# b41sh/pa

Measured on AMD Instinct MI355X. Metric: decoded GB/s (uncompressed) per node at 1/2/4/8 GPUs; bit-exact vs CPU, higher is better.
Workload: dtype int32

## Files before the change

include/strawboat_gpu.h:

```cpp
#ifndef STRAWBOAT_GPU_H
#define STRAWBOAT_GPU_H

#include <stddef.h>
#include <stdint.h>

#ifdef __cplusplus
extern "C" {
#endif

typedef enum {
  SB_OK = 0,
  SB_E_OUT_OF_SPEC = 1,
  SB_E_NYI = 2,
  SB_E_IO = 3,
  SB_E_CODEC = 4,
  SB_E_DEVICE = 5,
  SB_E_ARG = 6,
} sb_status;

typedef enum {
  SB_CODEC_NONE = 0,
  SB_CODEC_LZ4 = 1,
  SB_CODEC_ZSTD = 2,
  SB_CODEC_SNAPPY = 3,
// ... 222 lines not shown
                                       const sb_write_options* opts, uint64_t max_page_rows, uint8_t* d_out,
                                       uint64_t out_capacity, uint64_t* out_len, sb_page_meta* h_metas,
                                       uint64_t metas_cap, uint64_t* n_pages);
typedef struct {
  const int64_t* d_offsets;
  const uint8_t* d_validity;
} sb_nest_dev;
uint64_t sb_encode_nested_device_bound(const sb_nested_desc* desc, uint64_t n_rows, uint64_t n_level_bound,
                                       uint64_t n_leaf, uint64_t values_len, uint64_t max_page_rows);
sb_status sb_encode_nested_column_device(sb_ctx* ctx, const sb_nested_desc* desc, const sb_nest_dev* d_nests,
                                         const void* d_values, const int64_t* d_leaf_offsets, uint64_t values_len,
                                         const uint8_t* d_leaf_validity, uint64_t n_rows,
                                         const sb_write_options* opts, uint64_t max_page_rows, uint8_t* d_out,
                                         uint64_t out_capacity, uint64_t* out_len, sb_page_meta* h_metas,
                                         uint64_t metas_cap, uint64_t* n_pages);
sb_status sb_write_footer(const uint8_t* h_schema, uint64_t schema_len, const uint64_t* h_col_offsets,
                          const uint64_t* h_col_npages, uint64_t n_cols, const sb_page_meta* h_pages,
                          uint8_t** h_out, uint64_t* out_len);
void sb_free(void* p);

#define SB_LEAF_STRUCT 1u
#define SB_LEAF_MAP 2u
#define SB_LEAF_FIXED_SIZE_LIST 4u
#define SB_LEAF_UNION 8u
#define SB_LEAF_TOO_DEEP 16u
typedef struct {
  char name[64];
  int32_t arrow_type;
  int32_t physical_type;
  int32_t nullable;
  int32_t depth;
  int32_t list_nullable[SB_MAX_NEST];
  int32_t large_list[SB_MAX_NEST];
  uint32_t flags;
  int32_t top_field;
  uint32_t struct_mask;
  uint32_t map_mask;
  int32_t nest_id[SB_MAX_NEST];
} sb_leaf_info;

sb_status sb_parse_schema(const uint8_t* h_bytes, uint64_t len, sb_leaf_info* h_leaves, uint64_t cap,
                          uint64_t* n_leaves, uint64_t* n_fields);

typedef struct sb_file sb_file;
sb_status sb_file_open(const char* path, sb_file** out);
void sb_file_close(sb_file* f);
const char* sb_file_last_error(const sb_file* f);
uint64_t sb_file_num_columns(const sb_file* f);
sb_status sb_file_column(const sb_file* f, uint64_t col, uint64_t* offset, uint64_t* chunk_len, uint64_t* n_pages,
                         const sb_page_meta** h_pages);
sb_status sb_file_schema(const sb_file* f, const uint8_t** h_bytes, uint64_t* len);
sb_status sb_file_page_rows(sb_file* f, uint64_t col, uint64_t* h_rows, uint64_t cap);
sb_status sb_file_upload(sb_ctx* ctx, sb_file* f, uint64_t offset, uint64_t len, void* d_dst);

#ifdef __cplusplus
}
#endif
#endif
```

pa_amd/_native.py:

```python
from __future__ import annotations

import ctypes
import os
import subprocess

_HERE = os.path.dirname(os.path.abspath(__file__))
LIB_PATH = os.environ.get("PA_AMD_LIB") or os.path.join(_HERE, "libstrawboat_gpu.so")

OK, E_OUT_OF_SPEC, E_NYI, E_IO, E_CODEC, E_DEVICE, E_ARG = 0, 1, 2, 3, 4, 5, 6

INT8, INT16, INT32, INT64, UINT8, UINT16, UINT32, UINT64, FLOAT32, FLOAT64 = range(1, 11)
BOOLEAN = 15

EXPORTED = [
    "sb_ctx_create", "sb_ctx_destroy", "sb_ctx_set_stream", "sb_ctx_stream", "sb_ctx_device", "sb_sync", "sb_last_error",
    "sb_status_str", "sb_plan_column", "sb_plan_destroy", "sb_plan_num_rows", "sb_plan_num_pages",
    "sb_decode_planned", "sb_plan_status", "sb_decode_column", "sb_plan_last_kernel_ms", "sb_plan_enable_timing",
    "sb_decompress_values", "sb_read_meta", "sb_encode_page", "sb_encode_column", "sb_page_seed",
    "sb_write_footer", "sb_free", "sb_encode_binary_column", "sb_plan_values_bytes", "sb_decode_binary_planned",
    "sb_encode_list_column", "sb_plan_list_column", "sb_plan_num_leaves", "sb_decode_list_planned",
    "sb_encode_device_bound", "sb_encode_column_device", "sb_lz4_compress_host", "sb_snappy_compress_host", "sb_zstd_compress_host",
    "sb_encode_binary_device_bound", "sb_encode_binary_column_device", "sb_plan_nested_column",
    "sb_plan_nested_count", "sb_decode_nested_planned", "sb_parse_schema", "sb_file_open", "sb_file_close",
    "sb_file_last_error", "sb_file_num_columns", "sb_file_column", "sb_file_schema", "sb_file_upload",
    "sb_decode_page_validity", "sb_decode_page_levels", "sb_plan_column_at",
    "sb_encode_list_device_bound", "sb_encode_list_column_device", "sb_encode_nested_column",
    "sb_encode_nested_device_bound", "sb_encode_nested_column_device",
    "sb_select_create", "sb_select_num_rows", "sb_select_num_pages", "sb_select_page", "sb_select_destroy",
    "sb_plan_selected_column", "sb_decode_selected", "sb_decode_binary_selected", "sb_plan_selected_values_bytes",
    "sb_plan_selected_stats",
    "sb_list_page_rows", "sb_file_page_rows", "sb_plan_selected_list_column", "sb_decode_list_selected",
    "sb_plan_selected_leaves",
]

MAX_NEST = 4


class StrawboatError(RuntimeError):

    def __init__(self, status: int, msg: str):
        super().__init__(f"[{status}] {msg}")
        self.status = status


class PageMetaC(ctypes.Structure):
    _fields_ = [("length", ctypes.c_uint64), ("num_values", ctypes.c_uint64)]


class ColumnDescC(ctypes.Structure):
    _fields_ = [("physical_type", ctypes.c_int32), ("nullable", ctypes.c_int32)]


class WriteOptionsC(ctypes.Structure):
    _fields_ = [
        ("default_codec", ctypes.c_int32),
        ("has_ratio", ctypes.c_int32),
        ("ratio", ctypes.c_double),
        ("forbidden_mask", ctypes.c_uint32),
        ("forced_codec", ctypes.c_int32),
        ("seed", ctypes.c_uint64),
    ]


class LeafInfoC(ctypes.Structure):
    _fields_ = [("name", ctypes.c_char * 64), ("arrow_type", ctypes.c_int32), ("physical_type", ctypes.c_int32),
                ("nullable", ctypes.c_int32), ("depth", ctypes.c_int32), ("list_nullable", ctypes.c_int32 * MAX_NEST),
                ("large_list", ctypes.c_int32 * MAX_NEST), ("flags", ctypes.c_uint32), ("top_field", ctypes.c_int32),
                ("struct_mask", ctypes.c_uint32), ("map_mask", ctypes.c_uint32), ("nest_id", ctypes.c_int32 * MAX_NEST)]


class PrimitiveOutC(ctypes.Structure):
    _fields_ = [("d_values", ctypes.c_void_p), ("d_validity", ctypes.c_void_p)]


def build(force: bool = False) -> str:
    if force or not os.path.exists(LIB_PATH):
        subprocess.run(["make", "-s", "-C", _HERE], check=True)
    return LIB_PATH


_lib = None


def lib():
    global _lib
# ... 41 lines not shown
    L.sb_plan_enable_timing.restype = I32
    L.sb_plan_last_kernel_ms.argtypes = [P, P, ctypes.POINTER(ctypes.c_float)]
    L.sb_plan_last_kernel_ms.restype = I32
    L.sb_decompress_values.argtypes = [P, I32, P, U64, U64, P]
    L.sb_decompress_values.restype = I32
    L.sb_decode_page_validity.argtypes = [P, P, U64, U64, P, U64, ctypes.POINTER(U64)]
    L.sb_decode_page_validity.restype = I32
    L.sb_decode_page_levels.argtypes = [P, P, U64, U64, ctypes.c_uint32, ctypes.c_uint32, P, P,
                                        ctypes.POINTER(ctypes.c_uint32), ctypes.POINTER(U64)]
    L.sb_decode_page_levels.restype = I32
    L.sb_read_meta.argtypes = [P, U64, P, P, U64, P, U64, ctypes.POINTER(U64), ctypes.POINTER(U64)]
    L.sb_read_meta.restype = I32
    PU8 = ctypes.POINTER(ctypes.POINTER(ctypes.c_uint8))
    L.sb_encode_page.argtypes = [I32, P, P, U64, I32, ctypes.POINTER(WriteOptionsC), U64, PU8, ctypes.POINTER(U64)]
    L.sb_encode_page.restype = I32
    L.sb_encode_column.argtypes = [I32, P, P, U64, I32, ctypes.POINTER(WriteOptionsC), U64, I32, PU8,
                                   ctypes.POINTER(U64), ctypes.POINTER(ctypes.POINTER(PageMetaC)), ctypes.POINTER(U64)]
    L.sb_encode_column.restype = I32
    L.sb_encode_device_bound.argtypes = [I32, U64, I32, U64]
    L.sb_encode_device_bound.restype = U64
    L.sb_encode_column_device.argtypes = [P, I32, P, P, U64, I32, ctypes.POINTER(WriteOptionsC), U64, P, U64,
                                          ctypes.POINTER(U64), ctypes.POINTER(PageMetaC), U64, ctypes.POINTER(U64)]
    L.sb_encode_column_device.restype = I32
    L.sb_encode_list_device_bound.argtypes = [I32, U64, U64, I32, U64]
    L.sb_encode_list_device_bound.restype = U64
    L.sb_encode_list_column_device.argtypes = [P, I32, P, P, I32, P, P, I32, U64, ctypes.POINTER(WriteOptionsC), U64,
                                               P, U64, ctypes.POINTER(U64), ctypes.POINTER(PageMetaC), U64,
                                               ctypes.POINTER(U64)]
    L.sb_encode_list_column_device.restype = I32
    L.sb_page_seed.argtypes = [U64, U64]
    L.sb_page_seed.restype = U64
    L.sb_write_footer.argtypes = [P, U64, P, P, U64, P, PU8, ctypes.POINTER(U64)]
    L.sb_write_footer.restype = I32
    L.sb_free.argtypes = [P]
    L.sb_free.restype = None
    L.sb_parse_schema.argtypes = [P, U64, ctypes.POINTER(LeafInfoC), U64, ctypes.POINTER(U64), ctypes.POINTER(U64)]
    L.sb_parse_schema.restype = I32
    L.sb_file_open.argtypes = [ctypes.c_char_p, PP]
    L.sb_file_open.restype = I32
    L.sb_file_close.argtypes = [P]
    L.sb_file_close.restype = None
    L.sb_file_last_error.argtypes = [P]
    L.sb_file_last_error.restype = ctypes.c_char_p
    L.sb_file_num_columns.argtypes = [P]
    L.sb_file_num_columns.restype = U64
    L.sb_file_column.argtypes = [P, U64, ctypes.POINTER(U64), ctypes.POINTER(U64), ctypes.POINTER(U64),
                                 ctypes.POINTER(ctypes.POINTER(PageMetaC))]
    L.sb_file_column.restype = I32
    L.sb_file_schema.argtypes = [P, ctypes.POINTER(ctypes.POINTER(ctypes.c_uint8)), ctypes.POINTER(U64)]
    L.sb_file_schema.restype = I32
    L.sb_file_upload.argtypes = [P, P, U64, U64, P]
    L.sb_file_upload.restype = I32
    PU64 = ctypes.POINTER(U64)
    L.sb_select_create.argtypes = [P, P, U64, ctypes.POINTER(PageMetaC), U64, PP]
    L.sb_select_create.restype = I32
    L.sb_select_num_rows.argtypes = [P]
    L.sb_select_num_rows.restype = U64
    L.sb_select_num_pages.argtypes = [P]
    L.sb_select_num_pages.restype = U64
    L.sb_select_page.argtypes = [P, U64, PU64, PU64]
    L.sb_select_page.restype = I32
    L.sb_select_destroy.argtypes = [P]
    L.sb_select_destroy.restype = None
    L.sb_plan_selected_column.argtypes = [P, ctypes.POINTER(ColumnDescC), P, P, U64, I32, PP]
    L.sb_plan_selected_column.restype = I32
    L.sb_decode_selected.argtypes = [P, P, ctypes.POINTER(PrimitiveOutC)]
    L.sb_decode_selected.restype = I32
    L.sb_decode_binary_selected.argtypes = [P, P, P]
    L.sb_decode_binary_selected.restype = I32
    L.sb_plan_selected_values_bytes.argtypes = [P, P, PU64]
    L.sb_plan_selected_values_bytes.restype = I32
    L.sb_plan_selected_stats.argtypes = [P, PU64, PU64, PU64]
    L.sb_plan_selected_stats.restype = I32
    L.sb_list_page_rows.argtypes = [P, P, U64, ctypes.POINTER(PageMetaC), U64, PU64]
    L.sb_list_page_rows.restype = I32
    L.sb_file_page_rows.argtypes = [P, U64, PU64, U64]
    L.sb_file_page_rows.restype = I32
    L.sb_plan_selected_list_column.argtypes = [P, P, P, ctypes.POINTER(PageMetaC), U64, P, U64, I32, PP]
    L.sb_plan_selected_list_column.restype = I32
    L.sb_decode_list_selected.argtypes = [P, P, P]
    L.sb_decode_list_selected.restype = I32
    L.sb_plan_selected_leaves.argtypes = [P, P, PU64]
    L.sb_plan_selected_leaves.restype = I32
    _lib = L
    return L
```

pa_amd/csrc/sb_file.cpp:

```cpp
#include <hip/hip_runtime.h>

#include <fcntl.h>
#include <sys/stat.h>
#include <unistd.h>

#include <algorithm>
#include <cstring>
#include <mutex>
#include <string>
#include <thread>
#include <vector>

#include "../../include/strawboat_gpu.h"

namespace {

struct Fb {
  const uint8_t* b;
  uint64_t n;
  bool ok = true;

  template <class T>
  T rd(uint64_t p) {
    T v{};
    if (p > n || sizeof(T) > n - p) {
      ok = false;
      return v;
    }
    memcpy(&v, b + p, sizeof(T));
    return v;
  }
  uint64_t field(uint64_t t, int i) {
    const int64_t vt = (int64_t)t - (int64_t)rd<int32_t>(t);
    if (vt < 0 || (uint64_t)vt >= n) {
      ok = false;
      return 0;
    }
    const uint16_t vsz = rd<uint16_t>((uint64_t)vt);
    if ((uint64_t)(4 + 2 * i) + 2 > vsz) return 0;
    const uint16_t o = rd<uint16_t>((uint64_t)vt + 4 + 2 * i);
    return o ? t + o : 0;
  }
  uint64_t deref(uint64_t p) { return p + rd<uint32_t>(p); }
  uint64_t table(uint64_t t, int i) {
    const uint64_t f = field(t, i);
    return f ? deref(f) : 0;
  }
  template <class T>
  T scalar(uint64_t t, int i, T dflt) {
    const uint64_t f = field(t, i);
    return f ? rd<T>(f) : dflt;
  }
  uint64_t vec(uint64_t t, int i, uint32_t* len) {
    const uint64_t f = field(t, i);
    *len = 0;
    if (!f) return 0;
    const uint64_t v = deref(f);
    *len = rd<uint32_t>(v);
    if ((uint64_t)*len * 4 > n) ok = false;
    return v + 4;
  }
  std::string str(uint64_t t, int i) {
    uint32_t len;
    const uint64_t p = vec(t, i, &len);
    if (!p || p > n || len > n - p) return std::string();
    return std::string((const char*)b + p, len);
// ... 127 lines not shown
  return fb.ok && !w.fail;
}

bool parse_meta(const uint8_t* m, uint64_t len, std::vector<uint64_t>& col_off, std::vector<uint64_t>& col_start,
                std::vector<sb_page_meta>& pages) {
  uint64_t pos = 0;
  auto rd = [&](uint64_t* v) {
    if (pos + 8 > len) return false;
    memcpy(v, m + pos, 8);
    pos += 8;
    return true;
  };
  uint64_t nc;
  if (!rd(&nc) || nc > len / 16) return false;
  for (uint64_t c = 0; c < nc; c++) {
    uint64_t off, np;
    if (!rd(&off) || !rd(&np) || np > len / 16) return false;
    col_off.push_back(off);
    col_start.push_back(pages.size());
    for (uint64_t i = 0; i < np; i++) {
      sb_page_meta pm;
      if (!rd(&pm.length) || !rd(&pm.num_values)) return false;
      pages.push_back(pm);
    }
  }
  col_start.push_back(pages.size());
  return true;
}

bool pread_all(int fd, uint8_t* dst, uint64_t len, uint64_t off) {
  while (len) {
    const ssize_t r = ::pread(fd, dst, len, (off_t)off);
    if (r <= 0) return false;
    dst += r;
    len -= (uint64_t)r;
    off += (uint64_t)r;
  }
  return true;
}

}

struct sb_file {
  int fd = -1;
  uint64_t size = 0;
  std::vector<uint8_t> schema;
  std::vector<uint64_t> col_off, col_start;
  std::vector<sb_page_meta> pages;
  std::string err;
};

namespace {
constexpr uint64_t kFooterPreRead = 64 * 1024;
constexpr uint64_t kStageChunk = 16ull << 20;
constexpr int kReadThreads = 8;
constexpr int kMaxDevices = 64;

struct Staging {
  std::mutex mu;
  bool ready = false;
  uint8_t* pin[2] = {nullptr, nullptr};
  hipStream_t copy = nullptr;
  hipEvent_t ev[2] = {nullptr, nullptr};
  hipEvent_t done = nullptr;
  hipEvent_t before = nullptr;
  bool pending[2] = {false, false};
};
Staging g_staging[kMaxDevices];

bool staging_init(Staging& s) {
  if (s.ready) return true;
  bool ok = hipStreamCreateWithFlags(&s.copy, hipStreamNonBlocking) == hipSuccess &&
            hipEventCreateWithFlags(&s.done, hipEventDisableTiming) == hipSuccess &&
            hipEventCreateWithFlags(&s.before, hipEventDisableTiming) == hipSuccess;
  for (int k = 0; k < 2 && ok; k++)
    ok = hipHostMalloc((void**)&s.pin[k], kStageChunk, hipHostMallocDefault) == hipSuccess &&
         hipEventCreateWithFlags(&s.ev[k], hipEventDisableTiming) == hipSuccess;
  s.ready = ok;
  return ok;
}

sb_status file_fail(sb_file* f, sb_status st, const std::string& what) {
  if (f) f->err = what;
  return st;
}
}

extern "C" {

sb_status sb_parse_schema(const uint8_t* h_bytes, uint64_t len, sb_leaf_info* h_leaves, uint64_t cap,
                          uint64_t* n_leaves, uint64_t* n_fields) {
  if (!h_bytes || !n_leaves) return SB_E_ARG;
  std::vector<sb_leaf_info> v;
  if (!parse_schema(h_bytes, len, v, n_fields)) return SB_E_OUT_OF_SPEC;
  *n_leaves = v.size();
  if (h_leaves) memcpy(h_leaves, v.data(), std::min<uint64_t>(cap, v.size()) * sizeof(sb_leaf_info));
  return SB_OK;
}

sb_status sb_file_open(const char* path, sb_file** out) {
  if (!path || !out) return SB_E_ARG;
  *out = nullptr;
  const int fd = ::open(path, O_RDONLY);
  if (fd < 0) return SB_E_IO;
  sb_file* f = new sb_file();
  f->fd = fd;
  struct stat st;
  if (fstat(fd, &st) != 0 || st.st_size < 16) {
    sb_file_close(f);
    return SB_E_IO;
  }
  f->size = (uint64_t)st.st_size;
  std::vector<uint8_t> tail(std::min(f->size, kFooterPreRead));
  if (!pread_all(fd, tail.data(), tail.size(), f->size - tail.size())) {
    sb_file_close(f);
    return SB_E_IO;
  }
  uint32_t schema_size, meta_size;
  memcpy(&schema_size, tail.data() + tail.size() - 16, 4);
  memcpy(&meta_size, tail.data() + tail.size() - 12, 4);
  const uint64_t footer = 16ull + meta_size + schema_size;
  if (footer > f->size) {
    sb_file_close(f);
    return SB_E_OUT_OF_SPEC;
  }
  if (footer > tail.size()) {
    tail.resize(footer);
    if (!pread_all(fd, tail.data(), footer, f->size - footer)) {
      sb_file_close(f);
      return SB_E_IO;
    }
  }
  const uint8_t* end = tail.data() + tail.size();
  const uint8_t* meta = end - 16 - meta_size;
  f->schema.assign(meta - schema_size, meta);
  if (!parse_meta(meta, meta_size, f->col_off, f->col_start, f->pages)) {
    sb_file_close(f);
// ... 9 lines not shown
  delete f;
}

const char* sb_file_last_error(const sb_file* f) { return f ? f->err.c_str() : "null file"; }

uint64_t sb_file_num_columns(const sb_file* f) { return f ? f->col_off.size() : 0; }

sb_status sb_file_column(const sb_file* f, uint64_t col, uint64_t* offset, uint64_t* chunk_len, uint64_t* n_pages,
                         const sb_page_meta** h_pages) {
  if (!f || col >= f->col_off.size()) return SB_E_ARG;
  const uint64_t a = f->col_start[col], b = f->col_start[col + 1];
  uint64_t len = 0;
  for (uint64_t i = a; i < b; i++) {
    if (f->pages[i].length > f->size || len > f->size - f->pages[i].length) return SB_E_OUT_OF_SPEC;
    len += f->pages[i].length;
  }
  if (f->col_off[col] > f->size || len > f->size - f->col_off[col]) return SB_E_OUT_OF_SPEC;
  if (offset) *offset = f->col_off[col];
  if (chunk_len) *chunk_len = len;
  if (n_pages) *n_pages = b - a;
  if (h_pages) *h_pages = f->pages.data() + a;
  return SB_OK;
}

sb_status sb_file_schema(const sb_file* f, const uint8_t** h_bytes, uint64_t* len) {
  if (!f || !h_bytes || !len) return SB_E_ARG;
  *h_bytes = f->schema.data();
  *len = f->schema.size();
  return SB_OK;
}

sb_status sb_file_page_rows(sb_file* f, uint64_t col, uint64_t* h_rows, uint64_t cap) {
  if (!f || col >= f->col_off.size()) return SB_E_ARG;
  const uint64_t a = f->col_start[col], b = f->col_start[col + 1];
  if (b - a > cap || (b > a && !h_rows)) return file_fail(f, SB_E_ARG, "page rows: buffer too small");
  uint64_t pos = f->col_off[col];
  for (uint64_t i = a; i < b; i++) {
    const uint64_t len = f->pages[i].length;
    const std::string page = "page " + std::to_string(i - a);
    if (len < 12) return file_fail(f, SB_E_IO, page + ": shorter than a nested page's header");
    if (pos > f->size || f->size - pos < 4) return file_fail(f, SB_E_IO, page + " starts past the end of the file");
    uint8_t w[4];
    if (!pread_all(f->fd, w, 4, pos)) return file_fail(f, SB_E_IO, page + ": short read");
    h_rows[i - a] = (uint64_t)w[0] | (uint64_t)w[1] << 8 | (uint64_t)w[2] << 16 | (uint64_t)w[3] << 24;
    if (len > f->size) return file_fail(f, SB_E_IO, page + " reaches past the end of the file");
    pos += len;
  }
  return SB_OK;
}

sb_status sb_file_upload(sb_ctx* ctx, sb_file* f, uint64_t offset, uint64_t len, void* d_dst) {
  if (!ctx || !f || (!d_dst && len)) return SB_E_ARG;
  if (offset > f->size || len > f->size - offset) return file_fail(f, SB_E_IO, "range past the end of the file");
  const int dev = sb_ctx_device(ctx);
  if (dev < 0 || dev >= kMaxDevices || hipSetDevice(dev) != hipSuccess) return file_fail(f, SB_E_DEVICE, "device");
  Staging& sg = g_staging[dev];
  std::lock_guard<std::mutex> lock(sg.mu);
  if (!staging_init(sg)) return file_fail(f, SB_E_DEVICE, "staging buffers");
  uint8_t* dst = (uint8_t*)d_dst;
  if (len && (hipEventRecord(sg.before, (hipStream_t)sb_ctx_stream(ctx)) != hipSuccess ||
              hipStreamWaitEvent(sg.copy, sg.before, 0) != hipSuccess))
    return file_fail(f, SB_E_DEVICE, "stream order");
  for (uint64_t done = 0, k = 0; done < len; k++) {
    const int b = (int)(k & 1);
    const uint64_t n = std::min(kStageChunk, len - done);
    if (sg.pending[b] && hipEventSynchronize(sg.ev[b]) != hipSuccess)
      return file_fail(f, SB_E_DEVICE, "staging event");
    sg.pending[b] = false;
    const uint64_t part = (n + kReadThreads - 1) / kReadThreads;
    bool ok[kReadThreads];
    std::vector<std::thread> th;
    for (int t = 0; t < kReadThreads; t++) {
      const uint64_t a = std::min(n, t * part), e = std::min(n, a + part);
      ok[t] = true;
      if (e > a) th.emplace_back([&, t, a, e] { ok[t] = pread_all(f->fd, sg.pin[b] + a, e - a, offset + done + a); });
    }
    for (auto& x : th) x.join();
    for (int t = 0; t < kReadThreads; t++)
      if (!ok[t]) return file_fail(f, SB_E_IO, "short read");
    if (hipMemcpyAsync(dst + done, sg.pin[b], n, hipMemcpyHostToDevice, sg.copy) != hipSuccess ||
        hipEventRecord(sg.ev[b], sg.copy) != hipSuccess)
      return file_fail(f, SB_E_DEVICE, "staging copy");
    sg.pending[b] = true;
    done += n;
  }
  if (hipEventRecord(sg.done, sg.copy) != hipSuccess ||
      hipStreamWaitEvent((hipStream_t)sb_ctx_stream(ctx), sg.done, 0) != hipSuccess)
    return file_fail(f, SB_E_DEVICE, "stream join");
  return SB_OK;
}

}
```

pa_amd/select.py:

```python
from __future__ import annotations

import ctypes
import re
from typing import List, Optional, Sequence, Tuple

import numpy as np

from . import _native as N
from .binary import BINARY, LARGE_BINARY, LARGE_UTF8, UTF8, BinaryOutC, _ow
from .read import PageMeta, _as_device_bytes, physical_type, resolve_context

_BINARY_TYPES = (BINARY, LARGE_BINARY, UTF8, LARGE_UTF8)


def _error(st: int, msg: str) -> N.StrawboatError:
    e = N.StrawboatError(st, msg)
    m = re.search(r"\bpage (\d+)", msg)
    e.page = int(m.group(1)) if m else None
    return e


def normalize_ranges(ranges: Sequence[Tuple[int, int]], n_rows: int) -> List[Tuple[int, int]]:
    rs = []
    for a, b in ranges:
# ... 311 lines not shown

    def decode_async(self, offsets=None, list_validity=None, values=None, leaf_validity=None):
        from .nested import ListOutC

        if offsets is None:
            offsets, list_validity, values, leaf_validity = self.alloc_outputs()
        p = lambda t: None if t is None else t.data_ptr()
        out = ListOutC(p(offsets), p(list_validity), p(values), p(leaf_validity))
        st = N.lib().sb_decode_list_selected(self.ctx._h, self._h, ctypes.byref(out))
        if st:
            raise _error(st, self.ctx.error())
        return offsets, list_validity, values, leaf_validity

    def written_leaves(self) -> int:
        n = ctypes.c_uint64()
        st = N.lib().sb_plan_selected_leaves(self.ctx._h, self._h, ctypes.byref(n))
        if st:
            raise _error(st, self.ctx.error())
        return n.value

    def decode(self, *outs):
        o, lv, v, fv = self.decode_async(*outs)
        self.check()
        return o[: self.num_rows + 1], lv, v[: self.written_leaves()], fv

    def close(self):
        super().close()
        if getattr(self, "_own_resolved", False):
            self.resolved.close()
            self._own_resolved = False


def read_selected_list(chunk, page_metas: Sequence[PageMeta], dtype, list_nullable: bool, item_nullable: bool,
                       selection, ctx=None, large: bool = False, packed: bool = False):
    dec = SelectedListDecoder(chunk, page_metas, dtype, list_nullable, item_nullable, selection, ctx, large, packed)
    try:
        return dec.decode()
    finally:
        dec.close()


def read_selected(chunk, page_metas: Sequence[PageMeta], dtype_or_physical_type, nullable: bool, selection,
                  ctx=None, packed: bool = False):
    if isinstance(dtype_or_physical_type, int) and dtype_or_physical_type in _BINARY_TYPES:
        dec = SelectedBinaryDecoder(chunk, page_metas, dtype_or_physical_type, nullable, selection, ctx, packed)
    else:
        dec = SelectedColumnDecoder(chunk, page_metas, dtype_or_physical_type, nullable, selection, ctx, packed)
    try:
        return dec.decode()
    finally:
        dec.close()


def file_read_selected(f, col: int, selection: Selection, ctx=None):
    import torch

    from .file import _DTYPE

    if not 0 <= col < f.num_columns or len(f.leaves) != f.num_columns:
        raise N.StrawboatError(N.E_ARG, f"column {col} out of range")
    leaf = f.leaves[col]
    if leaf.depth:
        raise N.StrawboatError(N.E_NYI, f"leaf {leaf.name}: row selection of a nested leaf is not implemented")
    if leaf.flags or not leaf.physical_type:
        raise N.StrawboatError(N.E_NYI, f"leaf {leaf.name}: {leaf.arrow_type} has no page path here")
    ctx = resolve_context(ctx, selection.bitmap)
    cm = f.columns[col]
    res = selection.resolve(cm.pages, ctx)
    try:
        runs = res.runs()
        total = sum(r[1] for r in runs)
        buf = torch.empty(max(total, 1), dtype=torch.uint8, device=f"cuda:{ctx.device}")
        pos = 0
        for off, ln, _, _ in runs:
            f._check(N.lib().sb_file_upload(ctx._h, f._h, cm.offset + off, ln, ctypes.c_void_p(buf.data_ptr() + pos)))
            pos += ln
        f.last_uploaded_bytes = total
        pt = leaf.physical_type
        what = pt if pt in _BINARY_TYPES else _DTYPE[pt]
        return read_selected(buf[:max(total, 1)], cm.pages, what, leaf.nullable, res, ctx, packed=True)
    finally:
        res.close()


def file_read_selected_list(f, col: int, selection: Selection, ctx=None):
    import torch

    from .file import _DTYPE

    if not 0 <= col < f.num_columns or len(f.leaves) != f.num_columns:
        raise N.StrawboatError(N.E_ARG, f"column {col} out of range")
    leaf = f.leaves[col]
    if leaf.depth != 1 or leaf.flags or leaf.struct_mask or leaf.map_mask or leaf.physical_type not in _DTYPE \
            or _DTYPE[leaf.physical_type] == np.bool_:
        raise N.StrawboatError(N.E_NYI, f"leaf {leaf.name}: row selection takes one List / LargeList nest over a "
                                        f"fixed-width leaf")
    ctx = resolve_context(ctx, selection.bitmap)
    cm = f.columns[col]
    rows = f.page_rows(col)
    res = selection.resolve([PageMeta(m.length, r) for m, r in zip(cm.pages, rows)], ctx)
    try:
        runs = res.runs()
        total = sum(r[1] for r in runs)
        buf = torch.empty(max(total, 1), dtype=torch.uint8, device=f"cuda:{ctx.device}")
        pos = 0
        for off, ln, _, _ in runs:
            f._check(N.lib().sb_file_upload(ctx._h, f._h, cm.offset + off, ln, ctypes.c_void_p(buf.data_ptr() + pos)))
            pos += ln
        f.last_uploaded_bytes = total
        return read_selected_list(buf[:max(total, 1)], cm.pages, _DTYPE[leaf.physical_type], leaf.list_nullable[0],
                                  leaf.nullable, res, ctx, large=leaf.large_list[0], packed=True)
    finally:
        res.close()
```

rust/strawboat-gpu/src/ffi.rs:

```rust
#![allow(non_camel_case_types)]
use std::os::raw::{c_char, c_int, c_void};

#[repr(C)] pub struct sb_ctx { _p: [u8; 0] }
#[repr(C)] pub struct sb_plan { _p: [u8; 0] }
#[repr(C)] pub struct sb_file { _p: [u8; 0] }
#[repr(C)] pub struct sb_select { _p: [u8; 0] }

pub const SB_MAX_NEST: usize = 4;

#[repr(C)] #[derive(Clone, Copy)]
pub struct sb_leaf_info {
    pub name: [c_char; 64], pub arrow_type: i32, pub physical_type: i32, pub nullable: i32, pub depth: i32,
    pub list_nullable: [i32; SB_MAX_NEST], pub large_list: [i32; SB_MAX_NEST], pub flags: u32, pub top_field: i32,
    pub struct_mask: u32, pub map_mask: u32, pub nest_id: [i32; SB_MAX_NEST],
}

#[repr(C)] #[derive(Debug, Clone, Copy, PartialEq, Eq)]
pub struct sb_page_meta { pub length: u64, pub num_values: u64 }

#[repr(C)] #[derive(Clone, Copy)]
pub struct sb_column_desc { pub physical_type: i32, pub nullable: i32 }

#[repr(C)]
pub struct sb_primitive_out { pub d_values: *mut c_void, pub d_validity: *mut u8 }
// ... 119 lines not shown
    pub fn sb_encode_list_device_bound(physical_type: i32, n_rows: u64, n_child: u64, item_nullable: i32,
                                       max_page_rows: u64) -> u64;
    pub fn sb_encode_list_column_device(ctx: *mut sb_ctx, physical_type: i32, d_offsets: *const i64,
                                        d_list_validity: *const u8, list_nullable: i32, d_child: *const c_void,
                                        d_child_validity: *const u8, item_nullable: i32, n_rows: u64,
                                        opts: *const sb_write_options, max_page_rows: u64, d_out: *mut u8,
                                        out_capacity: u64, out_len: *mut u64, metas: *mut sb_page_meta,
                                        metas_cap: u64, n_pages: *mut u64) -> i32;
    pub fn sb_encode_nested_device_bound(desc: *const sb_nested_desc, n_rows: u64, n_level_bound: u64, n_leaf: u64,
                                         values_len: u64, max_page_rows: u64) -> u64;
    pub fn sb_encode_nested_column_device(ctx: *mut sb_ctx, desc: *const sb_nested_desc, d_nests: *const sb_nest_dev,
                                          d_values: *const c_void, d_leaf_offsets: *const i64, values_len: u64,
                                          d_leaf_validity: *const u8, n_rows: u64, opts: *const sb_write_options,
                                          max_page_rows: u64, d_out: *mut u8, out_capacity: u64, out_len: *mut u64,
                                          metas: *mut sb_page_meta, metas_cap: u64, n_pages: *mut u64) -> i32;
    pub fn sb_encode_page(physical_type: i32, values: *const c_void, validity: *const u8, n: u64,
                          nullable: i32, opts: *const sb_write_options, seed: u64, out: *mut *mut u8,
                          out_len: *mut u64) -> i32;
    pub fn sb_page_seed(seed: u64, page: u64) -> u64;
    pub fn sb_lz4_compress_host(src: *const u8, n: u64, dst: *mut u8) -> u64;
    pub fn sb_snappy_compress_host(src: *const u8, n: u64, dst: *mut u8) -> u64;
    pub fn sb_zstd_compress_host(src: *const u8, n: u64, dst: *mut u8) -> u64;
    pub fn sb_decompress_values(ctx: *mut sb_ctx, physical_type: i32, d_stream: *const u8, stream_len: u64,
                                length: u64, d_out: *mut c_void) -> i32;
    pub fn sb_decode_page_validity(ctx: *mut sb_ctx, d_page: *const u8, page_len: u64, length: u64,
                                   d_validity: *mut u32, bit_offset: u64, consumed: *mut u64) -> i32;
    pub fn sb_decode_page_levels(ctx: *mut sb_ctx, d_page: *const u8, page_len: u64, num_levels: u64,
                                 max_rep_level: u32, max_def_level: u32, d_rep: *mut u16, d_def: *mut u16,
                                 rows: *mut u32, consumed: *mut u64) -> i32;
    pub fn sb_ctx_device(ctx: *const sb_ctx) -> i32;
    pub fn sb_plan_enable_timing(plan: *mut sb_plan, on: i32) -> i32;
    pub fn sb_plan_last_kernel_ms(ctx: *mut sb_ctx, plan: *mut sb_plan, ms: *mut f32) -> i32;
    pub fn sb_write_footer(schema: *const u8, schema_len: u64, col_offsets: *const u64,
                           col_npages: *const u64, n_cols: u64, pages: *const sb_page_meta,
                           out: *mut *mut u8, out_len: *mut u64) -> i32;
    pub fn sb_read_meta(file: *const u8, len: u64, col_offsets: *mut u64, col_page_start: *mut u64,
                        cols_cap: u64, pages: *mut sb_page_meta, pages_cap: u64,
                        n_cols: *mut u64, n_pages: *mut u64) -> i32;
    pub fn sb_free(p: *mut c_void);
    pub fn sb_ctx_stream(ctx: *mut sb_ctx) -> *mut c_void;
    pub fn sb_status_str(status: c_int) -> *const c_char;
    pub fn sb_plan_num_pages(plan: *const sb_plan) -> u64;
    pub fn sb_parse_schema(bytes: *const u8, len: u64, leaves: *mut sb_leaf_info, cap: u64,
                           n_leaves: *mut u64, n_fields: *mut u64) -> i32;
    pub fn sb_file_open(path: *const c_char, out: *mut *mut sb_file) -> i32;
    pub fn sb_file_close(f: *mut sb_file);
    pub fn sb_file_last_error(f: *const sb_file) -> *const c_char;
    pub fn sb_file_num_columns(f: *const sb_file) -> u64;
    pub fn sb_file_column(f: *const sb_file, col: u64, offset: *mut u64, chunk_len: *mut u64, n_pages: *mut u64,
                          pages: *mut *const sb_page_meta) -> i32;
    pub fn sb_file_schema(f: *const sb_file, bytes: *mut *const u8, len: *mut u64) -> i32;
    pub fn sb_file_page_rows(f: *mut sb_file, col: u64, rows: *mut u64, cap: u64) -> i32;
    pub fn sb_file_upload(ctx: *mut sb_ctx, f: *mut sb_file, offset: u64, len: u64, d_dst: *mut c_void) -> i32;
}

#[link(name = "amdhip64")]
extern "C" {
    pub fn hipMalloc(ptr: *mut *mut c_void, size: usize) -> c_int;
    pub fn hipFree(ptr: *mut c_void) -> c_int;
    pub fn hipMemcpy(dst: *mut c_void, src: *const c_void, size: usize, kind: c_int) -> c_int;
    pub fn hipMemsetAsync(dst: *mut c_void, value: c_int, size: usize, stream: *mut c_void) -> c_int;
    pub fn hipSetDevice(device: c_int) -> c_int;
    pub fn hipGetDevice(device: *mut c_int) -> c_int;
}
pub const HIP_MEMCPY_HOST_TO_DEVICE: c_int = 1;
pub const HIP_MEMCPY_DEVICE_TO_HOST: c_int = 2;
```

Baseline: 4480.

## Replace double-buffered file staging with multi-slot reader ring and batched range upload

Replaces the two 16 MiB pinned staging buffers, which were filled by per-chunk spawned-and-joined thread teams, with a 32 MiB pinned ring of 1 MiB slots. A persistent reader team pulls blocks while the caller coalesces filled slots into async host-to-device copies and retires them via per-slot events. This lets disk reads overlap with copies continuously instead of in lockstep. It also adds a batched sb_file_upload_ranges call so selected-page runs upload in one pipelined pass instead of one call per run. The cost is more threads (12 readers), more events and more synchronisation complexity.

Result: no change. 4492, median of 3 (+0.3%).

```diff
diff --git a/include/strawboat_gpu.h b/include/strawboat_gpu.h
--- a/include/strawboat_gpu.h
+++ b/include/strawboat_gpu.h
@@ -298,6 +298,8 @@
 sb_status sb_file_schema(const sb_file* f, const uint8_t** h_bytes, uint64_t* len);
 sb_status sb_file_page_rows(sb_file* f, uint64_t col, uint64_t* h_rows, uint64_t cap);
 sb_status sb_file_upload(sb_ctx* ctx, sb_file* f, uint64_t offset, uint64_t len, void* d_dst);
+sb_status sb_file_upload_ranges(sb_ctx* ctx, sb_file* f, const uint64_t* offsets, const uint64_t* lens, uint64_t n,
+                                void* d_dst);
 
 #ifdef __cplusplus
 }
diff --git a/pa_amd/_native.py b/pa_amd/_native.py
--- a/pa_amd/_native.py
+++ b/pa_amd/_native.py
@@ -30,7 +30,7 @@
     "sb_plan_selected_column", "sb_decode_selected", "sb_decode_binary_selected", "sb_plan_selected_values_bytes",
     "sb_plan_selected_stats",
     "sb_list_page_rows", "sb_file_page_rows", "sb_plan_selected_list_column", "sb_decode_list_selected",
-    "sb_plan_selected_leaves",
+    "sb_plan_selected_leaves", "sb_file_upload_ranges",
 ]
 
 MAX_NEST = 4
@@ -178,6 +178,8 @@
     L.sb_file_upload.argtypes = [P, P, U64, U64, P]
     L.sb_file_upload.restype = I32
     PU64 = ctypes.POINTER(U64)
+    L.sb_file_upload_ranges.argtypes = [P, P, PU64, PU64, U64, P]
+    L.sb_file_upload_ranges.restype = I32
     L.sb_select_create.argtypes = [P, P, U64, ctypes.POINTER(PageMetaC), U64, PP]
     L.sb_select_create.restype = I32
     L.sb_select_num_rows.argtypes = [P]
diff --git a/pa_amd/csrc/sb_file.cpp b/pa_amd/csrc/sb_file.cpp
--- a/pa_amd/csrc/sb_file.cpp
+++ b/pa_amd/csrc/sb_file.cpp
@@ -5,13 +5,15 @@
 #include <unistd.h>
 
 #include <algorithm>
+#include <cstdio>
+#include <cstdlib>
 #include <cstring>
 #include <mutex>
 #include <string>
-#include <thread>
 #include <vector>
 
 #include "../../include/strawboat_gpu.h"
+#include "sb_upload_ring.h"
 
 namespace {
 
@@ -245,30 +247,54 @@
 
 namespace {
 constexpr uint64_t kFooterPreRead = 64 * 1024;
-constexpr uint64_t kStageChunk = 16ull << 20;
-constexpr int kReadThreads = 8;
+constexpr uint64_t kStageBytes = 32ull << 20;
+constexpr uint64_t kStageBlock = 1ull << 20;
+constexpr int kReadThreads = 12;
+constexpr int kMaxReadThreads = 16;
+constexpr int kMaxSlots = 128;
 constexpr int kMaxDevices = 64;
+
+struct Tuning {
+  uint64_t block = kStageBlock;
+  int slots = (int)(kStageBytes / kStageBlock);
+  int readers = kReadThreads;
+  bool phases = false;
+};
+const Tuning& tuning() {
+  static const Tuning t = [] {
+    Tuning v;
+    if (const char* e = getenv("SB_UPLOAD_READERS")) v.readers = std::min(kMaxReadThreads, std::max(1, atoi(e)));
+    if (const char* e = getenv("SB_UPLOAD_BLOCK_KIB")) {
+      const int k = atoi(e);
+      if (k >= 256 && k <= 16384 && (k & (k - 1)) == 0) v.block = (uint64_t)k << 10;
+    }
+    v.slots = (int)(kStageBytes / v.block);
+    if (const char* e = getenv("SB_UPLOAD_PHASES")) v.phases = atoi(e) != 0;
+    return v;
+  }();
+  return t;
+}
 
 struct Staging {
   std::mutex mu;
   bool ready = false;
-  uint8_t* pin[2] = {nullptr, nullptr};
+  uint8_t* pin = nullptr;
   hipStream_t copy = nullptr;
-  hipEvent_t ev[2] = {nullptr, nullptr};
+  hipEvent_t ev[kMaxSlots] = {};
   hipEvent_t done = nullptr;
   hipEvent_t before = nullptr;
-  bool pending[2] = {false, false};
+  sb_ring::State ring;
 };
 Staging g_staging[kMaxDevices];
 
 bool staging_init(Staging& s) {
   if (s.ready) return true;
-  bool ok = hipStreamCreateWithFlags(&s.copy, hipStreamNonBlocking) == hipSuccess &&
-            hipEventCreateWithFlags(&s.done, hipEventDisableTiming) == hipSuccess &&
-            hipEventCreateWithFlags(&s.before, hipEventDisableTiming) == hipSuccess;
-  for (int k = 0; k < 2 && ok; k++)
-    ok = hipHostMalloc((void**)&s.pin[k], kStageChunk, hipHostMallocDefault) == hipSuccess &&
-         hipEventCreateWithFlags(&s.ev[k], hipEventDisableTiming) == hipSuccess;
+  bool ok = (s.copy || hipStreamCreateWithFlags(&s.copy, hipStreamNonBlocking) == hipSuccess) &&
+            (s.done || hipEventCreateWithFlags(&s.done, hipEventDisableTiming) == hipSuccess) &&
+            (s.before || hipEventCreateWithFlags(&s.before, hipEventDisableTiming) == hipSuccess) &&
+            (s.pin || hipHostMalloc((void**)&s.pin, kStageBytes, hipHostMallocDefault) == hipSuccess);
+  for (int k = 0; k < tuning().slots && ok; k++)
+    ok = s.ev[k] || hipEventCreateWithFlags(&s.ev[k], hipEventDisableTiming) == hipSuccess;
   s.ready = ok;
   return ok;
 }
@@ -276,6 +302,70 @@
 sb_status file_fail(sb_file* f, sb_status st, const std::string& what) {
   if (f) f->err = what;
   return st;
+}
+
+struct HipCopier {
+  Staging& sg;
+  uint8_t* dst;
+  uint64_t block;
+  const char* what = "staging copy";
+  bool enqueue(int slot, uint64_t n, uint64_t o) {
+    what = "staging copy";
+    if (hipMemcpyAsync(dst + o, sg.pin + (uint64_t)slot * block, n, hipMemcpyHostToDevice, sg.copy) != hipSuccess)
+      return false;
+    if (hipEventRecord(sg.ev[slot], sg.copy) != hipSuccess) {
+      (void)hipStreamSynchronize(sg.copy);
+      return false;
+    }
+    return true;
+  }
+  bool wait(int slot) {
+    what = "staging event";
+    return hipEventSynchronize(sg.ev[slot]) == hipSuccess;
+  }
+};
+
+sb_status upload_segments(sb_ctx* ctx, sb_file* f, const sb_ring::Segment* segs, size_t nseg, uint64_t total,
+                          void* d_dst) {
+  const int dev = sb_ctx_device(ctx);
+  if (dev < 0 || dev >= kMaxDevices || hipSetDevice(dev) != hipSuccess) return file_fail(f, SB_E_DEVICE, "device");
+  Staging& sg = g_staging[dev];
+  std::lock_guard<std::mutex> lock(sg.mu);
+  if (!staging_init(sg)) return file_fail(f, SB_E_DEVICE, "staging buffers");
+  if (!total) return SB_OK;
+  const hipStream_t stream = (hipStream_t)sb_ctx_stream(ctx);
+  if (hipEventRecord(sg.before, stream) != hipSuccess || hipStreamWaitEvent(sg.copy, sg.before, 0) != hipSuccess)
+    return file_fail(f, SB_E_DEVICE, "stream order");
+  const Tuning& tn = tuning();
+  sb_ring::Phases ph;
+  sb_ring::Config cfg;
+  cfg.block = tn.block;
+  cfg.slots = tn.slots;
+  cfg.readers = tn.readers;
+  cfg.phases = tn.phases ? &ph : nullptr;
+  HipCopier cp{sg, (uint8_t*)d_dst, tn.block};
+  const uint64_t t0 = tn.phases ? sb_ring::detail::now_ns() : 0;
+  int st;
+  try {
+    st = sb_ring::upload(sg.ring, sg.pin, cfg, f->fd, segs, nseg, cp);
+  } catch (...) {
+    return file_fail(f, SB_E_DEVICE, "staging ring");
+  }
+  if (tn.phases)
+    fprintf(stderr,
+            "sb_upload_phases {\"bytes\": %llu, \"block\": %llu, \"slots\": %d, \"readers\": %llu, \"blocks\": %llu, "
+            "\"copies\": %llu, \"call_us\": %.1f, \"team_create_us\": %.1f, \"reader_slot_wait_us\": %.1f, "
+            "\"reader_pread_us\": %.1f, \"caller_fill_wait_us\": %.1f, \"caller_copy_wait_us\": %.1f, "
+            "\"caller_enqueue_us\": %.1f}\n",
+            (unsigned long long)total, (unsigned long long)tn.block, tn.slots, (unsigned long long)ph.threads,
+            (unsigned long long)ph.blocks, (unsigned long long)ph.copies, (sb_ring::detail::now_ns() - t0) / 1e3,
+            ph.team_ns / 1e3, ph.slot_wait_ns / 1e3, ph.pread_ns / 1e3, ph.fill_wait_ns / 1e3, ph.copy_wait_ns / 1e3,
+            ph.enqueue_ns / 1e3);
+  if (st == sb_ring::kIo) return file_fail(f, SB_E_IO, "short read");
+  if (st != sb_ring::kOk) return file_fail(f, SB_E_DEVICE, cp.what);
+  if (hipEventRecord(sg.done, sg.copy) != hipSuccess || hipStreamWaitEvent(stream, sg.done, 0) != hipSuccess)
+    return file_fail(f, SB_E_DEVICE, "stream join");
+  return SB_OK;
 }
 }
 
@@ -391,42 +481,24 @@
 sb_status sb_file_upload(sb_ctx* ctx, sb_file* f, uint64_t offset, uint64_t len, void* d_dst) {
   if (!ctx || !f || (!d_dst && len)) return SB_E_ARG;
   if (offset > f->size || len > f->size - offset) return file_fail(f, SB_E_IO, "range past the end of the file");
-  const int dev = sb_ctx_device(ctx);
-  if (dev < 0 || dev >= kMaxDevices || hipSetDevice(dev) != hipSuccess) return file_fail(f, SB_E_DEVICE, "device");
-  Staging& sg = g_staging[dev];
-  std::lock_guard<std::mutex> lock(sg.mu);
-  if (!staging_init(sg)) return file_fail(f, SB_E_DEVICE, "staging buffers");
-  uint8_t* dst = (uint8_t*)d_dst;
-  if (len && (hipEventRecord(sg.before, (hipStream_t)sb_ctx_stream(ctx)) != hipSuccess ||
-              hipStreamWaitEvent(sg.copy, sg.before, 0) != hipSuccess))
-    return file_fail(f, SB_E_DEVICE, "stream order");
-  for (uint64_t done = 0, k = 0; done < len; k++) {
-    const int b = (int)(k & 1);
-    const uint64_t n = std::min(kStageChunk, len - done);
-    if (sg.pending[b] && hipEventSynchronize(sg.ev[b]) != hipSuccess)
-      return file_fail(f, SB_E_DEVICE, "staging event");
-    sg.pending[b] = false;
-    const uint64_t part = (n + kReadThreads - 1) / kReadThreads;
-    bool ok[kReadThreads];
-    std::vector<std::thread> th;
-    for (int t = 0; t < kReadThreads; t++) {
-      const uint64_t a = std::min(n, t * part), e = std::min(n, a + part);
-      ok[t] = true;
-      if (e > a) th.emplace_back([&, t, a, e] { ok[t] = pread_all(f->fd, sg.pin[b] + a, e - a, offset + done + a); });
-    }
-    for (auto& x : th) x.join();
-    for (int t = 0; t < kReadThreads; t++)
-      if (!ok[t]) return file_fail(f, SB_E_IO, "short read");
-    if (hipMemcpyAsync(dst + done, sg.pin[b], n, hipMemcpyHostToDevice, sg.copy) != hipSuccess ||
-        hipEventRecord(sg.ev[b], sg.copy) != hipSuccess)
-      return file_fail(f, SB_E_DEVICE, "staging copy");
-    sg.pending[b] = true;
-    done += n;
-  }
-  if (hipEventRecord(sg.done, sg.copy) != hipSuccess ||
-      hipStreamWaitEvent((hipStream_t)sb_ctx_stream(ctx), sg.done, 0) != hipSuccess)
-    return file_fail(f, SB_E_DEVICE, "stream join");
-  return SB_OK;
-}
-
-}
+  const sb_ring::Segment seg{offset, len};
+  return upload_segments(ctx, f, &seg, 1, len, d_dst);
+}
+
+sb_status sb_file_upload_ranges(sb_ctx* ctx, sb_file* f, const uint64_t* offsets, const uint64_t* lens, uint64_t n,
+                                void* d_dst) {
+  if (!ctx || !f || (n && (!offsets || !lens))) return SB_E_ARG;
+  std::vector<sb_ring::Segment> segs;
+  segs.reserve(n);
+  uint64_t total = 0;
+  for (uint64_t i = 0; i < n; i++) {
+    if (offsets[i] > f->size || lens[i] > f->size - offsets[i] || lens[i] > UINT64_MAX - total)
+      return file_fail(f, SB_E_IO, "range past the end of the file");
+    total += lens[i];
+    if (lens[i]) segs.push_back({offsets[i], lens[i]});
+  }
+  if (!d_dst && total) return SB_E_ARG;
+  return upload_segments(ctx, f, segs.data(), segs.size(), total, d_dst);
+}
+
+}
diff --git a/pa_amd/csrc/sb_upload_ring.h b/pa_amd/csrc/sb_upload_ring.h
--- /dev/null
+++ b/pa_amd/csrc/sb_upload_ring.h
@@ -0,0 +1,285 @@
+#pragma once
+
+#include <errno.h>
+#include <unistd.h>
+
+#include <algorithm>
+#include <atomic>
+#include <chrono>
+#include <condition_variable>
+#include <cstdint>
+#include <deque>
+#include <mutex>
+#include <system_error>
+#include <thread>
+#include <vector>
+
+namespace sb_ring {
+
+struct Segment {
+  uint64_t off, len;
+};
+
+enum Status { kOk = 0, kIo = 1, kCopy = 2 };
+
+struct Phases {
+  uint64_t team_ns = 0;
+  uint64_t slot_wait_ns = 0;
+  uint64_t pread_ns = 0;
+  uint64_t fill_wait_ns = 0;
+  uint64_t copy_wait_ns = 0;
+  uint64_t enqueue_ns = 0;
+  uint64_t threads = 0, blocks = 0, copies = 0;
+};
+
+struct Config {
+  uint64_t block = 0;
+  int slots = 0;
+  int readers = 1;
+  Phases* phases = nullptr;
+  std::atomic<int>* live = nullptr;
+};
+
+struct State {
+  struct Run {
+    int slot, count;
+  };
+  uint64_t head = 0;
+  uint64_t busy = 0;
+  std::deque<Run> inflight;
+};
+
+namespace detail {
+
+inline uint64_t now_ns() {
+  return (uint64_t)std::chrono::duration_cast<std::chrono::nanoseconds>(
+             std::chrono::steady_clock::now().time_since_epoch())
+      .count();
+}
+
+inline bool pread_all(int fd, uint8_t* dst, uint64_t len, uint64_t off) {
+  while (len) {
+    const ssize_t r = ::pread(fd, dst, len, (off_t)off);
+    if (r < 0 && errno == EINTR) continue;
+    if (r <= 0) return false;
+    dst += r;
+    len -= (uint64_t)r;
+    off += (uint64_t)r;
+  }
+  return true;
+}
+
+inline bool read_packed(int fd, const Segment* segs, const std::vector<uint64_t>& start, uint64_t pos, uint64_t n,
+                        uint8_t* dst) {
+  size_t j = (size_t)(std::upper_bound(start.begin(), start.end(), pos) - start.begin()) - 1;
+  while (n) {
+    const uint64_t in = pos - start[j], take = std::min(n, segs[j].len - in);
+    if (take && !pread_all(fd, dst, take, segs[j].off + in)) return false;
+    dst += take;
+    pos += take;
+    n -= take;
+    j++;
+  }
+  return true;
+}
+
+template <class Copier>
+struct Call {
+  State& st;
+  uint8_t* stage;
+  const Config& cfg;
+  int fd;
+  const Segment* segs;
+  Copier& cp;
+  std::vector<uint64_t> start;
+  uint64_t total = 0, nblocks = 0, head0 = 0;
+
+  std::mutex mu;
+  std::condition_variable cv_caller, cv_slot;
+  std::atomic<uint64_t> next{0};
+  std::atomic<int> err{kOk};
+  std::vector<uint8_t> filled;
+  uint64_t limit = 0;
+  int waiting = 0;
+  bool stop = false;
+  uint64_t r_slot_ns = 0, r_pread_ns = 0;
+
+  Call(State& s, uint8_t* stg, const Config& c, int f, const Segment* sg, size_t nseg, Copier& k)
+      : st(s), stage(stg), cfg(c), fd(f), segs(sg), cp(k), start(nseg + 1, 0) {
+    for (size_t j = 0; j < nseg; j++) start[j + 1] = start[j] + segs[j].len;
+    total = start[nseg];
+    nblocks = (total + cfg.block - 1) / cfg.block;
+    head0 = st.head;
+  }
+
+  int slot_of(uint64_t i) const { return (int)((head0 + i) % (uint64_t)cfg.slots); }
+  uint64_t bytes_of(uint64_t i, uint64_t k) const { return std::min(total, (i + k) * cfg.block) - i * cfg.block; }
+
+  bool read_block(uint64_t i) {
+    return read_packed(fd, segs, start, i * cfg.block, bytes_of(i, 1), stage + (uint64_t)slot_of(i) * cfg.block);
+  }
+
+  bool retire_front() {
+    const State::Run run = st.inflight.front();
+    st.inflight.pop_front();
+    st.busy -= (uint64_t)run.count;
+    const uint64_t t0 = cfg.phases ? now_ns() : 0;
+    const bool ok = cp.wait(run.slot);
+    if (cfg.phases) cfg.phases->copy_wait_ns += now_ns() - t0;
+    return ok;
+  }
+
+  bool enqueue(uint64_t i, uint64_t k) {
+    const uint64_t t0 = cfg.phases ? now_ns() : 0;
+    const bool ok = cp.enqueue(slot_of(i), bytes_of(i, k), i * cfg.block);
+    if (cfg.phases) {
+      cfg.phases->enqueue_ns += now_ns() - t0;
+      cfg.phases->copies++;
+    }
+    if (!ok) return false;
+    st.inflight.push_back({slot_of(i), (int)k});
+    st.busy += k;
+    st.head += k;
+    return true;
+  }
+
+  int run_inline() {
+    for (uint64_t i = 0; i < nblocks; i++) {
+      while (st.busy >= (uint64_t)cfg.slots)
+        if (!retire_front()) return kCopy;
+      const uint64_t t0 = cfg.phases ? now_ns() : 0;
+      const bool ok = read_block(i);
+      if (cfg.phases) cfg.phases->pread_ns += now_ns() - t0;
+      if (!ok) return kIo;
+      if (!enqueue(i, 1)) return kCopy;
+    }
+    return kOk;
+  }
+
+  void fail(int e) {
+    int none = kOk;
+    err.compare_exchange_strong(none, e);
+    cv_slot.notify_all();
+    cv_caller.notify_all();
+  }
+
+  void reader() {
+    if (cfg.live) cfg.live->fetch_add(1);
+    uint64_t slot_ns = 0, pread_ns = 0;
+    while (err.load() == kOk) {
+      const uint64_t i = next.fetch_add(1);
+      if (i >= nblocks) break;
+      {
+        std::unique_lock<std::mutex> lk(mu);
+        if (i >= limit && !stop && err.load() == kOk) {
+          const uint64_t t0 = cfg.phases ? now_ns() : 0;
+          waiting++;
+          cv_caller.notify_one();
+          cv_slot.wait(lk, [&] { return i < limit || stop || err.load() != kOk; });
+          waiting--;
+          if (cfg.phases) slot_ns += now_ns() - t0;
+        }
+        if (stop || err.load() != kOk) break;
+      }
+      const uint64_t t0 = cfg.phases ? now_ns() : 0;
+      const bool ok = read_block(i);
+      if (cfg.phases) pread_ns += now_ns() - t0;
+      std::lock_guard<std::mutex> lk(mu);
+      if (!ok) {
+        fail(kIo);
+        break;
+      }
+      filled[i] = 1;
+      cv_caller.notify_one();
+    }
+    {
+      std::lock_guard<std::mutex> lk(mu);
+      r_slot_ns += slot_ns;
+      r_pread_ns += pread_ns;
+    }
+    if (cfg.live) cfg.live->fetch_sub(1);
+  }
+
+  struct Team {
+    Call& c;
+    std::vector<std::thread> th;
+    explicit Team(Call& call) : c(call) {}
+    ~Team() {
+      {
+        std::lock_guard<std::mutex> lk(c.mu);
+        c.stop = true;
+        c.cv_slot.notify_all();
+      }
+      for (auto& t : th) t.join();
+    }
+  };
+
+  int run_team(int nthreads) {
+    filled.assign(nblocks, 0);
+    limit = (uint64_t)cfg.slots - st.busy;
+    const uint64_t max_run = std::max<uint64_t>(1, (uint64_t)cfg.slots / 4);
+    uint64_t enq = 0;
+    {
+      Team team(*this);
+      const uint64_t t0 = cfg.phases ? now_ns() : 0;
+      team.th.reserve((size_t)nthreads);
+      try {
+        for (int t = 0; t < nthreads; t++) team.th.emplace_back([this] { reader(); });
+      } catch (const std::system_error&) {
+      }
+      if (cfg.phases) {
+        cfg.phases->team_ns += now_ns() - t0;
+        cfg.phases->threads += team.th.size();
+      }
+      if (team.th.empty()) return run_inline();
+      std::unique_lock<std::mutex> lk(mu);
+      while (enq < nblocks && err.load() == kOk) {
+        if (filled[enq]) {
+          uint64_t k = 1;
+          while (k < max_run && enq + k < nblocks && filled[enq + k] && slot_of(enq) + (int)k < cfg.slots) k++;
+          lk.unlock();
+          const bool ok = enqueue(enq, k);
+          lk.lock();
+          if (!ok) {
+            fail(kCopy);
+            break;
+          }
+          enq += k;
+        } else if (waiting > 0 && !st.inflight.empty()) {
+          const uint64_t n = (uint64_t)st.inflight.front().count;
+          lk.unlock();
+          const bool ok = retire_front();
+          lk.lock();
+          limit += n;
+          cv_slot.notify_all();
+          if (!ok) {
+            fail(kCopy);
+            break;
+          }
+        } else {
+          const uint64_t t1 = cfg.phases ? now_ns() : 0;
+          cv_caller.wait(lk);
+          if (cfg.phases) cfg.phases->fill_wait_ns += now_ns() - t1;
+        }
+      }
+    }
+    if (cfg.phases) {
+      cfg.phases->slot_wait_ns += r_slot_ns;
+      cfg.phases->pread_ns += r_pread_ns;
+    }
+    return err.load();
+  }
+};
+
+}
+
+template <class Copier>
+int upload(State& st, uint8_t* stage, const Config& cfg, int fd, const Segment* segs, size_t nseg, Copier& cp) {
+  detail::Call<Copier> c(st, stage, cfg, fd, segs, nseg, cp);
+  if (!c.total) return kOk;
+  if (cfg.phases) cfg.phases->blocks += c.nblocks;
+  const int n = (int)std::min<uint64_t>((uint64_t)std::max(1, cfg.readers), c.nblocks);
+  return c.nblocks == 1 ? c.run_inline() : c.run_team(n);
+}
+
+}
diff --git a/pa_amd/select.py b/pa_amd/select.py
--- a/pa_amd/select.py
+++ b/pa_amd/select.py
@@ -387,6 +387,13 @@
         dec.close()
 
 
+def _upload_runs(f, ctx, base: int, runs, buf) -> None:
+    n = len(runs)
+    offs = (ctypes.c_uint64 * max(n, 1))(*[base + r[0] for r in runs])
+    lens = (ctypes.c_uint64 * max(n, 1))(*[r[1] for r in runs])
+    f._check(N.lib().sb_file_upload_ranges(ctx._h, f._h, offs, lens, n, ctypes.c_void_p(buf.data_ptr())))
+
+
 def file_read_selected(f, col: int, selection: Selection, ctx=None):
     import torch
 
@@ -406,10 +413,7 @@
         runs = res.runs()
         total = sum(r[1] for r in runs)
         buf = torch.empty(max(total, 1), dtype=torch.uint8, device=f"cuda:{ctx.device}")
-        pos = 0
-        for off, ln, _, _ in runs:
-            f._check(N.lib().sb_file_upload(ctx._h, f._h, cm.offset + off, ln, ctypes.c_void_p(buf.data_ptr() + pos)))
-            pos += ln
+        _upload_runs(f, ctx, cm.offset, runs, buf)
         f.last_uploaded_bytes = total
         pt = leaf.physical_type
         what = pt if pt in _BINARY_TYPES else _DTYPE[pt]
@@ -438,10 +442,7 @@
         runs = res.runs()
         total = sum(r[1] for r in runs)
         buf = torch.empty(max(total, 1), dtype=torch.uint8, device=f"cuda:{ctx.device}")
-        pos = 0
-        for off, ln, _, _ in runs:
-            f._check(N.lib().sb_file_upload(ctx._h, f._h, cm.offset + off, ln, ctypes.c_void_p(buf.data_ptr() + pos)))
-            pos += ln
+        _upload_runs(f, ctx, cm.offset, runs, buf)
         f.last_uploaded_bytes = total
         return read_selected_list(buf[:max(total, 1)], cm.pages, _DTYPE[leaf.physical_type], leaf.list_nullable[0],
                                   leaf.nullable, res, ctx, large=leaf.large_list[0], packed=True)
diff --git a/rust/strawboat-gpu/src/ffi.rs b/rust/strawboat-gpu/src/ffi.rs
--- a/rust/strawboat-gpu/src/ffi.rs
+++ b/rust/strawboat-gpu/src/ffi.rs
@@ -195,6 +195,8 @@
     pub fn sb_file_schema(f: *const sb_file, bytes: *mut *const u8, len: *mut u64) -> i32;
     pub fn sb_file_page_rows(f: *mut sb_file, col: u64, rows: *mut u64, cap: u64) -> i32;
     pub fn sb_file_upload(ctx: *mut sb_ctx, f: *mut sb_file, offset: u64, len: u64, d_dst: *mut c_void) -> i32;
+    pub fn sb_file_upload_ranges(ctx: *mut sb_ctx, f: *mut sb_file, offsets: *const u64, lens: *const u64, n: u64,
+                                 d_dst: *mut c_void) -> i32;
 }
 
 #[link(name = "amdhip64")]
```
